# aszepieniec/stark-anatomy

Hardware: NVIDIA H100
Metric: 128-bit field butterflies/sec on 2^20 NTT (higher is better)
Workload: dtype u128 mod p (4x u32 limbs, Montgomery)

## Files before the change

### stark-anatomy_b200/csrc/ntt_tile.cuh

```cuda
#pragma once
#include "field.cuh"

namespace sa {

constexpr int TILE_MAX_PEERS = 7;

struct TileArgs {
    const fe *in;
    fe *out;
    const fe *tw;
    const fe *twb;
    long long in_sr, in_sc, in_sb;
    long long out_sr, out_sc, out_sb;
    long long twb_stride;
    long long in_sb2, out_sb2;
    int inner;
    int ncols;
    int nbatch;
    int has_scale;
    fe scale;
    fe cst[8];
    fe *peer_out[TILE_MAX_PEERS];
    int npeer;
    fe *mc_out;
};

enum { TF_FULL = 1, TF_TWB = 2, TF_SCALE = 4, TF_DYNAMIC = 8, TF_PEERS = 16 };

template <int LOGL, int ELOG, int C>
struct TilePlan {
    static constexpr int L = 1 << LOGL;
    static constexpr int EL = LOGL >= ELOG ? ELOG : LOGL;
    static constexpr int E = 1 << EL;
    static constexpr int NFULL = LOGL / EL;
    static constexpr int REM = LOGL % EL;
    static constexpr int NST = NFULL + (REM ? 1 : 0);
    static constexpr int NLOOP = NST - 1;
    static constexpr int LASTLOG = REM ? REM : EL;
    static constexpr int TPT = (L / E) * C;
    static constexpr int TPC = TPT >= 128 ? 1 : 128 / TPT;
    static constexpr int THREADS = TPT * TPC;
    static constexpr size_t TILE_BYTES = (size_t)TPC * L * C * sizeof(fe);
    static constexpr size_t TW_BYTES = (size_t)L * sizeof(fe);
    SA_HDC size_t smem_bytes() { return NST > 1 ? TILE_BYTES + TW_BYTES + 16 : 0; }
};

SA_HDC int tile_tw_slot(int e) { return e ^ ((e >> 3) & 7); }

SA_HDC int tile_bitrev(int i, int r) {
    int j = 0;
    for (int b = 1, bb = r >> 1; b < r; b <<= 1, bb >>= 1)
        if (i & b) j |= bb;
    return j;
}

template <int R, int LEN>
SA_HD void dft_level(fe *x, const fe *cst, int cstep) {
    constexpr int HALF = LEN / 2, STEP = R / LEN;
#if defined(__CUDA_ARCH__)
#pragma unroll
#endif
    for (int g = 0; g < R; g += LEN) {
#if defined(__CUDA_ARCH__)
#pragma unroll
#endif
        for (int k = 0; k < HALF; k++) {
            const fe t = (k == 0) ? x[g + k + HALF] : fe_montmul(x[g + k + HALF], cst[k * STEP * cstep]);
            const fe e = x[g + k];
            x[g + k] = fe_add(e, t);
            x[g + k + HALF] = fe_sub(e, t);
        }
    }
    if constexpr (LEN < R) dft_level<R, LEN * 2>(x, cst, cstep);
}

template <int R>
SA_HD void dft_regs(fe *x, const fe *cst, int cstep) {
#if defined(__CUDA_ARCH__)
#pragma unroll
#endif
// ... 58 lines not shown
#endif
}

SA_HD long long tile_batch_offset(long long b, int inner, long long sb, long long sb2) {
    return inner <= 1 ? b * sb : (b / inner) * sb + (b % inner) * sb2;
}

#if defined(__CUDA_ARCH__)
__device__ __forceinline__ void tile_stage_twiddles(fe *dst, const fe *src, uint32_t bytes, uint64_t *bar) {
    const uint32_t bar_a = (uint32_t)__cvta_generic_to_shared(bar);
    const uint32_t dst_a = (uint32_t)__cvta_generic_to_shared(dst);
    asm volatile("mbarrier.init.shared::cta.b64 [%0], 1;" ::"r"(bar_a));
    asm volatile("fence.mbarrier_init.release.cluster;" ::: "memory");
    asm volatile("mbarrier.arrive.expect_tx.shared::cta.b64 _, [%0], %1;" ::"r"(bar_a), "r"(bytes) : "memory");
    asm volatile("cp.async.bulk.shared::cluster.global.mbarrier::complete_tx::bytes [%0], [%1], %2, [%3];" ::"r"(dst_a),
                 "l"(src), "r"(bytes), "r"(bar_a)
                 : "memory");
}
__device__ __forceinline__ void tile_wait_twiddles(uint64_t *bar) {
    const uint32_t bar_a = (uint32_t)__cvta_generic_to_shared(bar);
    asm volatile(
        "{\n\t"
        ".reg .pred p;\n\t"
        "TW_WAIT_%=:\n\t"
        "mbarrier.try_wait.parity.shared::cta.b64 p, [%0], 0;\n\t"
        "@p bra TW_DONE_%=;\n\t"
        "bra TW_WAIT_%=;\n\t"
        "TW_DONE_%=:\n\t"
        "}" ::"r"(bar_a)
        : "memory");
}
#endif

template <int LOGL, int ELOG, int C, int FLAGS>
SA_HD void ntt_tile_full_stage(int t, fe *sm, const TileArgs &a, long long b, int col0, bool valid, bool first,
                               int ml, const fe *tw, uint64_t *bar) {
    using P = TilePlan<LOGL, ELOG, C>;
    constexpr int R = P::E;
    constexpr int CSTEP = 16 / R;
    const int c = t % C, q = t / C;
    const int col = col0 + c;
    const bool active = (FLAGS & TF_FULL) ? true : (valid && col < a.ncols);
    const int M = 1 << ml, wlog = LOGL - ml - P::EL;
    const int K = q >> ml, m = q & (M - 1);
    const int row0 = (K << (ml + P::EL)) + m;
    fe x[R];
    if (first) {
        const fe *src = a.in + tile_batch_offset(b, a.inner, a.in_sb, a.in_sb2) + (long long)col * a.in_sc;
        const unsigned sr = (unsigned)a.in_sr, step = (unsigned)M * sr, off0 = (unsigned)row0 * sr;
#if defined(__CUDA_ARCH__)
#pragma unroll
#endif
        for (int d = 0; d < R; d++) x[d] = active ? tile_ld(src + (off0 + (unsigned)d * step)) : fe_zero();
    } else {
#if defined(__CUDA_ARCH__)
#pragma unroll
#endif
        for (int d = 0; d < R; d++) x[d] = tile_ld(sm + (row0 + d * M) * C + c);
    }
    dft_regs<R>(x, a.cst, CSTEP);
#if defined(__CUDA_ARCH__)
    extern __shared__ uint4 sa_smem_u4[];
    tw = reinterpret_cast<const fe *>(sa_smem_u4) + P::TILE_BYTES / sizeof(fe);
    if (first) tile_wait_twiddles(reinterpret_cast<uint64_t *>(const_cast<fe *>(tw) + P::L));
    (void)bar;
#else
    (void)bar;
#endif
    tile_st(sm + row0 * C + c, x[0]);
#if defined(__CUDA_ARCH__)
#pragma unroll
#endif
    for (int k = 1; k < R; k++) {
        const fe w = tile_ld(tw + tile_tw_slot((k * m) << wlog));
        tile_st(sm + (row0 + k * M) * C + c, fe_montmul(x[k], w));
    }
}

template <int LOGL, int ELOG, int C, int FLAGS>
SA_HD void ntt_tile_last_stage(int t, fe *sm, const TileArgs &a, long long b, int col0, bool valid) {
    using P = TilePlan<LOGL, ELOG, C>;
    constexpr int R = 1 << P::LASTLOG, U = P::E / R;
    constexpr bool FIRST = P::NST == 1;
    constexpr int CSTEP = LOGL >= 4 ? 16 / R : (1 << LOGL) / R;
    const int c = t % C, q = t / C;
    const int col = col0 + c;
    const bool active = (FLAGS & TF_FULL) ? true : (valid && col < a.ncols);
    const bool use_twb = (FLAGS & TF_DYNAMIC) ? (a.twb != nullptr) : ((FLAGS & TF_TWB) != 0);
    const bool use_scale = (FLAGS & TF_DYNAMIC) ? (a.has_scale != 0) : ((FLAGS & TF_SCALE) != 0);
    const fe *twb = use_twb ? a.twb + col : nullptr;
    const unsigned out_sr = (unsigned)a.out_sr, twb_sr = (unsigned)a.twb_stride;
    fe *dst = a.out + tile_batch_offset(b, a.inner, a.out_sb, a.out_sb2) + (long long)col * a.out_sc;
#if defined(__CUDA_ARCH__)
#pragma unroll 1
#endif
    for (int s = 0; s < U; s++) {
        const int row0 = (q * U + s) * R;
        fe x[R];
        if (FIRST) {
            const fe *src = a.in + tile_batch_offset(b, a.inner, a.in_sb, a.in_sb2) + (long long)col * a.in_sc;
#if defined(__CUDA_ARCH__)
#pragma unroll
#endif
            for (int d = 0; d < R; d++) x[d] = active ? tile_ld(src + (unsigned)(row0 + d) * (unsigned)a.in_sr) : fe_zero();
        } else {
#if defined(__CUDA_ARCH__)
#pragma unroll
#endif
            for (int d = 0; d < R; d++) x[d] = tile_ld(sm + (row0 + d) * C + c);
        }
        dft_regs<R>(x, a.cst, CSTEP);
#if defined(__CUDA_ARCH__)
#pragma unroll
#endif
        for (int k = 0; k < R; k++) {
            const unsigned o = (unsigned)tile_digit_reverse<LOGL, ELOG, C>(row0 + k);
            fe v = x[k];
            if (use_twb && active) v = fe_montmul(v, tile_ldg(twb + o * twb_sr));
            if (use_scale) v = fe_montmul(v, a.scale);
            if (active) {
                if constexpr ((FLAGS & TF_PEERS) != 0) {
                    const long long rel = (dst - a.out) + (long long)(o * out_sr);
                    if (a.mc_out != nullptr) {
                        tile_st_multicast(a.mc_out + rel, v);
                    } else {
                        tile_st(dst + o * out_sr, v);
                        for (int pi = 0; pi < a.npeer; pi++) tile_st(a.peer_out[pi] + rel, v);
                    }
                } else {
                    tile_st(dst + o * out_sr, v);
                }
            }
        }
    }
}

template <int LOGL, int ELOG, int C, int FLAGS = TF_DYNAMIC>
struct TileStages {
    using P = TilePlan<LOGL, ELOG, C>;
    SA_HD static void full(int st, int t, fe *sm, const TileArgs &a, long long b, int col0, bool valid,
                           const fe *tw, uint64_t *bar) {
        ntt_tile_full_stage<LOGL, ELOG, C, FLAGS>(t, sm, a, b, col0, valid, st == 0, LOGL - (st + 1) * P::EL, tw,
                                                   bar);
    }
    SA_HD static void last(int t, fe *sm, const TileArgs &a, long long b, int col0, bool valid) {
        ntt_tile_last_stage<LOGL, ELOG, C, FLAGS>(t, sm, a, b, col0, valid);
    }
};

template <int LOGL, int ELOG, int C>
SA_HD int tile_variant(const TileArgs &a) {
    using P = TilePlan<LOGL, ELOG, C>;
    const long long tiles = (long long)((a.ncols + C - 1) / C) * a.nbatch;
    const int peers = (a.npeer > 0 || a.mc_out != nullptr) ? TF_PEERS : 0;
    if (LOGL < 5 || a.ncols % C != 0 || tiles % P::TPC != 0 || a.has_scale) return TF_DYNAMIC | peers;
    if (peers) return a.twb == nullptr ? (TF_FULL | TF_PEERS) : (TF_DYNAMIC | TF_PEERS);
    return TF_FULL | (a.twb != nullptr ? TF_TWB : 0);
}

}
```

### stark-anatomy_b200/csrc/sa_b200.cu

```cuda
#include <cuda_runtime.h>
#include <pthread.h>
#include <sched.h>

#include <algorithm>
#include <atomic>
#include <cctype>
#include <chrono>
#include <cstdio>
#include <cstdlib>
#include <cstring>
#include <map>
#include <memory>
#include <mutex>
#include <string>
#include <tuple>
#include <vector>

#include "../../include/sa_b200.h"
#include "field.cuh"
#include "fri_merkle.cuh"
#include "hash.cuh"
#include "ntt_plan.cuh"
#include "ntt_tile.cuh"

// ... 26 lines not shown
}
static inline bool host_is_pow2(size_t n) { return n && !(n & (n - 1)); }
static inline int host_log2(size_t n) {
    int l = 0;
    while ((size_t(1) << l) < n) l++;
    return l;
}

template <int LOGL, int ELOG, int C>
struct TileLaunch {
    using P = TilePlan<LOGL, ELOG, C>;
    static constexpr int TARGET = (P::EL <= 3 && LOGL > 3) ? 1024 : 512;
    static constexpr int MINB = TARGET / P::THREADS > 0 ? TARGET / P::THREADS : 1;
};

template <int LOGL, int ELOG, int C, int FLAGS>
__global__ void __launch_bounds__(TilePlan<LOGL, ELOG, C>::THREADS, TileLaunch<LOGL, ELOG, C>::MINB)
    ntt_tile_kernel(const __grid_constant__ TileArgs a, long long total_tiles, int tiles_per_batch) {
    using P = TilePlan<LOGL, ELOG, C>;
    using S = TileStages<LOGL, ELOG, C, FLAGS>;
    extern __shared__ uint4 sa_smem_u4[];
    fe *smem = reinterpret_cast<fe *>(sa_smem_u4);
    const int tic = threadIdx.x / P::TPT, t = threadIdx.x % P::TPT;
    const long long tile = (long long)blockIdx.x * P::TPC + tic;
    const bool valid = tile < total_tiles;
    const long long b = valid ? tile / tiles_per_batch : 0;
    const int col0 = valid ? (int)(tile % tiles_per_batch) * C : 0;
    fe *sm = smem + (size_t)tic * P::L * C;
    fe *tw = nullptr;
    uint64_t *bar = nullptr;
    asm volatile("griddepcontrol.launch_dependents;");
    if constexpr (P::NLOOP > 0) {
        tw = smem + P::TILE_BYTES / sizeof(fe);
        bar = reinterpret_cast<uint64_t *>(tw + P::L);
        if (threadIdx.x == 0) tile_stage_twiddles(tw, a.tw, (uint32_t)P::TW_BYTES, bar);
        __syncthreads();
    }
    asm volatile("griddepcontrol.wait;" ::: "memory");
#pragma unroll 1
    for (int st = 0; st < P::NLOOP; st++) {
        S::full(st, t, sm, a, b, col0, valid, tw, bar);
        __syncthreads();
    }
    S::last(t, sm, a, b, col0, valid);
}

__global__ void k_pow_table(fe *out, fe base_m, fe lead_m, long long count, int swz) {
    const long long e0 = ((long long)blockIdx.x * blockDim.x + threadIdx.x) * 16;
    if (e0 >= count) return;
    fe acc = fe_montmul(fe_mont_pow_u64(base_m, (uint64_t)e0), lead_m);
    for (int i = 0; i < 16 && e0 + i < count; i++) {
        const long long e = e0 + i;
        tile_st(out + (swz ? (long long)tile_tw_slot((int)e) : e), acc);
        acc = fe_montmul(acc, base_m);
    }
}
__global__ void k_twb_table(fe *out, fe w_m, fe scale_m, int n1, int n2) {
    const long long idx = (long long)blockIdx.x * blockDim.x + threadIdx.x;
    const long long per_row = (n2 + 15) / 16;
    const long long k = idx / per_row;
    const long long j0 = (idx % per_row) * 16;
    if (k >= n1) return;
    const fe wk = fe_mont_pow_u64(w_m, (uint64_t)k);
    fe acc = fe_montmul(fe_mont_pow_u64(wk, (uint64_t)j0), scale_m);
    for (int i = 0; i < 16 && j0 + i < n2; i++) {
        tile_st(out + k * n2 + j0 + i, acc);
        acc = fe_montmul(acc, wk);
    }
}

__global__ void k_pointwise_mul(fe *out, const fe *a, const fe *b, long long n) {
    const long long stride = (long long)gridDim.x * blockDim.x;
    for (long long i = (long long)blockIdx.x * blockDim.x + threadIdx.x; i < n; i += stride)
        tile_st(out + i, fe_montmul(fe_to_mont(tile_ld(a + i)), tile_ld(b + i)));
}
__global__ void k_pointwise_div(fe *out, const fe *a, const fe *b, long long n, int *zero_flag) {
    constexpr int G = 8;
    const long long stride = (long long)gridDim.x * blockDim.x;
    const long long i0 = (long long)blockIdx.x * blockDim.x + threadIdx.x;
    for (long long base = i0; base < n; base += stride * G) {
        fe bm[G], pre[G];
        fe acc = fe_mont_one();
#pragma unroll
        for (int g = 0; g < G; g++) {
            const long long i = base + g * stride;
            fe v = (i < n) ? tile_ld(b + i) : fe_one();
            if (fe_is_zero(v)) {
                *zero_flag = 1;
// ... 681 lines not shown
            if (it->second.tick < victim->second.tick) victim = it;
        g_cache_bytes -= victim->second.tables->bytes;
        g_cache.erase(victim);
    }
}
template <class T>
static std::shared_ptr<T> cache_find(const CacheKey &key) {
    cache_config();
    std::lock_guard<std::mutex> lock(g_plan_mu);
    auto it = g_cache.find(key);
    if (it == g_cache.end()) return nullptr;
    it->second.tick = ++g_cache_tick;
    return std::static_pointer_cast<T>(it->second.tables);
}
template <class T>
static std::shared_ptr<T> cache_publish(const CacheKey &key, std::shared_ptr<T> made) {
    std::lock_guard<std::mutex> lock(g_plan_mu);
    auto it = g_cache.find(key);
    if (it != g_cache.end()) {
        it->second.tick = ++g_cache_tick;
        return std::static_pointer_cast<T>(it->second.tables);
    }
    cache_make_room(made->bytes);
    CacheEntry e;
    e.tables = made;
    e.tick = ++g_cache_tick;
    g_cache.emplace(key, e);
    g_cache_bytes += made->bytes;
    return made;
}

static int build_pow_table(DeviceTables &owner, fe **out, const fe &base_m, const fe &lead_m, long long count,
                           cudaStream_t st, int swz = 0) {
    int rc = owner.alloc((void **)out, sizeof(fe) * (size_t)count);
    if (rc != SA_OK) return rc;
    const long long threads = (count + 15) / 16;
    const int bs = 128;
    k_pow_table<<<(unsigned)((threads + bs - 1) / bs), bs, 0, st>>>(*out, base_m, lead_m, count, swz);
    SA_LAUNCH_CHECK();
    return SA_OK;
}

static int get_plan(PlanPtr *plan_out, int log_n, const fe &root, int inverse, cudaStream_t st) {
    int dev = 0;
    SA_CUDA(cudaGetDevice(&dev));
    const uint64_t rlo = (uint64_t)root.v[0] | ((uint64_t)root.v[1] << 32);
    const uint64_t rhi = (uint64_t)root.v[2] | ((uint64_t)root.v[3] << 32);
    const CacheKey key(0, dev, (uint64_t)log_n, rlo, rhi, inverse ? 1 : 0);
    if ((*plan_out = cache_find<NttPlan>(key))) return SA_OK;
    const uint64_t n = 1ull << log_n;
    const fe root_m = fe_to_mont(root);
    if (!fe_eq(fe_mont_pow_u64(root_m, n), fe_mont_one())) return SA_EROOTORDER;
    if (fe_eq(fe_mont_pow_u64(root_m, n / 2), fe_mont_one())) return SA_ENOTPRIM;
    const fe w_m = inverse ? fe_mont_inv(root_m) : root_m;
    const fe ninv_m = fe_mont_inv(fe_to_mont(fe_from_u64(n)));
    PlanPtr made = std::make_shared<NttPlan>();
    NttPlan &p = *made;
    p.device = dev;
    p.log_n = log_n;
    int rc;
    const NttShape shape = ntt_shape(log_n);
    p.l1 = shape.l1;
    p.l2 = shape.l2;
    p.l3 = shape.l3;
    if (shape.l3 > 0) {
        const int n1 = 1 << p.l1, n2 = 1 << p.l2, n3 = 1 << p.l3;
        const long long m = (long long)n2 * n3;
        const fe w1_m = fe_mont_pow_u64(w_m, (uint64_t)m);
        const fe wsub_m = fe_mont_pow_u64(w_m, (uint64_t)n1);
        const fe w2_m = fe_mont_pow_u64(wsub_m, (uint64_t)n3);
        const fe w3_m = fe_mont_pow_u64(wsub_m, (uint64_t)n2);
        if ((rc = build_pow_table(p, &p.tw1, w1_m, fe_mont_one(), n1, st, 1)) != SA_OK) return rc;
// ... 73 lines not shown
    const int tiles_per_batch = (a.ncols + C - 1) / C;
    const long long total = (long long)tiles_per_batch * a.nbatch;
    const long long grid = (total + P::TPC - 1) / P::TPC;
    const size_t smem = P::smem_bytes();
    if (smem > 48 * 1024) {
        static std::atomic<bool> attr_done[SA_MAX_DEVICES];
        const int rc = optin_smem(ntt_tile_kernel<LOGL, ELOG, C, FLAGS>, attr_done, smem);
        if (rc != SA_OK) return rc;
    }
    static const bool pdl = !(getenv("SA_NTT_PDL") && atoi(getenv("SA_NTT_PDL")) == 0);
    if (pdl) {
        cudaLaunchConfig_t cfg = {};
        cfg.gridDim = dim3((unsigned)grid);
        cfg.blockDim = dim3(P::THREADS);
        cfg.dynamicSmemBytes = smem;
        cfg.stream = st;
        cudaLaunchAttribute attr[1];
        attr[0].id = cudaLaunchAttributeProgrammaticStreamSerialization;
        attr[0].val.programmaticStreamSerializationAllowed = 1;
        cfg.attrs = attr;
        cfg.numAttrs = 1;
        const int tpb = tiles_per_batch;
        SA_CUDA(cudaLaunchKernelEx(&cfg, ntt_tile_kernel<LOGL, ELOG, C, FLAGS>, a, total, tpb));
        g_launches.fetch_add(1, std::memory_order_relaxed);
        return SA_OK;
    }
    ntt_tile_kernel<LOGL, ELOG, C, FLAGS><<<(unsigned)grid, P::THREADS, smem, st>>>(a, total, tiles_per_batch);
    SA_LAUNCH_CHECK();
    return SA_OK;
}
template <int LOGL, int ELOG, int C>
static int launch_tile(const TileArgs &a, cudaStream_t st) {
    const int variant = tile_variant<LOGL, ELOG, C>(a);
    if constexpr (LOGL >= 5) {
        switch (variant) {
            case TF_FULL | TF_TWB: return launch_tile_variant<LOGL, ELOG, C, TF_FULL | TF_TWB>(a, st);
            case TF_FULL: return launch_tile_variant<LOGL, ELOG, C, TF_FULL>(a, st);
            case TF_FULL | TF_PEERS: return launch_tile_variant<LOGL, ELOG, C, TF_FULL | TF_PEERS>(a, st);
        }
    }
    if (variant & TF_PEERS) return launch_tile_variant<LOGL, ELOG, C, TF_DYNAMIC | TF_PEERS>(a, st);
    return launch_tile_variant<LOGL, ELOG, C, TF_DYNAMIC>(a, st);
}

static int g_tile_elog = -1, g_tile_c = -1;
static void tile_config() {
    if (g_tile_elog >= 0) return;
    const char *e = getenv("SA_NTT_ELOG"), *c = getenv("SA_NTT_C");
    g_tile_elog = e ? atoi(e) : 0;
    g_tile_c = c ? atoi(c) : 0;
}
template <int LOGL>
static int launch_tile_shape(const TileArgs &a, cudaStream_t st) {
    tile_config();
#ifdef SA_TUNE
    if (LOGL >= 9 && g_tile_elog > 0) {
        if (g_tile_elog == 3 && g_tile_c == 8) return launch_tile<LOGL, 3, 8>(a, st);
        if (g_tile_elog == 3 && g_tile_c == 4) return launch_tile<LOGL, 3, 4>(a, st);
        if (g_tile_elog == 3 && g_tile_c == 2) return launch_tile<LOGL, 3, 2>(a, st);
        if (g_tile_elog == 4 && g_tile_c == 4) return launch_tile<LOGL, 4, 4>(a, st);
        if (g_tile_elog == 4 && g_tile_c == 2) return launch_tile<LOGL, 4, 2>(a, st);
        if (g_tile_elog == 4 && g_tile_c == 8) return launch_tile<LOGL, 4, 8>(a, st);
    }
#endif
    if constexpr (LOGL >= 9) {
        static const int peer_c = [] {
// ... 1226 lines not shown
```

### stark-anatomy_b200/csrc/field.cuh

```cuda
#pragma once
#include <stdint.h>

#if defined(__CUDACC__)
#define SA_HD __host__ __device__ __forceinline__
#define SA_HDC __host__ __device__ static constexpr
#define SA_ALIGN16 __align__(16)
#else
#define SA_HD inline
#define SA_HDC static constexpr
#define SA_ALIGN16 alignas(16)
#endif

namespace sa {

struct SA_ALIGN16 fe {
    uint32_t v[4];
};

static constexpr uint32_t P3 = 0xCB800000u;

SA_HD fe fe_make(uint32_t a0, uint32_t a1, uint32_t a2, uint32_t a3) {
    fe r;
    r.v[0] = a0; r.v[1] = a1; r.v[2] = a2; r.v[3] = a3;
    return r;
// ... 102 lines not shown
    uint32_t ca = (uint32_t)(s >> 63);
    uint32_t cb = (u0 != 0u);
    u = (u >> 32) + (uint64_t)m1 * P3;
    uint32_t u1 = (uint32_t)u;
    u = (u >> 32) + (uint64_t)m2 * P3;
    uint32_t u2 = (uint32_t)u;
    u = (u >> 32) + (uint64_t)m3 * P3;
    uint32_t u3 = (uint32_t)u;
    uint32_t u4 = (uint32_t)(u >> 32);
    c = (uint64_t)t[4] + u1 + ca + cb;
    uint32_t r0 = (uint32_t)c;
    c = (c >> 32) + t[5] + u2;
    uint32_t r1 = (uint32_t)c;
    c = (c >> 32) + t[6] + u3;
    uint32_t r2 = (uint32_t)c;
    c = (c >> 32) + t[7] + u4;
    uint32_t r3 = (uint32_t)c;
    return fe_cond_sub_p_portable(r0, r1, r2, r3, (uint32_t)(c >> 32));
}

#if defined(__CUDA_ARCH__) && !defined(SA_PORTABLE_FIELD)
__device__ __forceinline__ fe fe_cond_sub_p(uint32_t r0, uint32_t r1, uint32_t r2, uint32_t r3, uint32_t top) {
    uint32_t d0, d1, d2, d3, br;
    asm("sub.cc.u32 %0, %5, 1;\n\t"
        "subc.cc.u32 %1, %6, 0;\n\t"
        "subc.cc.u32 %2, %7, 0;\n\t"
        "subc.cc.u32 %3, %8, 0xCB800000;\n\t"
        "subc.u32 %4, 0, 0;"
        : "=r"(d0), "=r"(d1), "=r"(d2), "=r"(d3), "=r"(br)
        : "r"(r0), "r"(r1), "r"(r2), "r"(r3));
    bool use = (top != 0) | (br == 0);
    return fe_make(use ? d0 : r0, use ? d1 : r1, use ? d2 : r2, use ? d3 : r3);
}
#ifndef SA_FIELD_MASK
#define SA_FIELD_MASK 1
#endif
#ifndef SA_MONTMUL_V
#define SA_MONTMUL_V 1
#endif
template <bool ALU_MASKS>
__device__ __forceinline__ fe fe_cond_add_p(uint32_t d0, uint32_t d1, uint32_t d2, uint32_t d3, uint32_t m) {
    uint32_t p0, p3;
    if (ALU_MASKS) {
        p0 = m & 1u;
        p3 = m & 0xCB800000u;
    } else {
        asm("mul.lo.u32 %0, %2, %2;\n\t"
            "mul.lo.u32 %1, %2, 0x34800000;"
            : "=r"(p0), "=r"(p3) : "r"(m));
    }
    uint32_t r0, r1, r2, r3;
    asm("add.cc.u32 %0, %4, %8;\n\t"
        "addc.cc.u32 %1, %5, 0;\n\t"
        "addc.cc.u32 %2, %6, 0;\n\t"
        "addc.u32 %3, %7, %9;"
        : "=r"(r0), "=r"(r1), "=r"(r2), "=r"(r3)
        : "r"(d0), "r"(d1), "r"(d2), "r"(d3), "r"(p0), "r"(p3));
    return fe_make(r0, r1, r2, r3);
}
__device__ __forceinline__ fe fe_add(const fe &a, const fe &b) {
    uint32_t s0, s1, s2, s3, c;
    asm("add.cc.u32 %0, %5, %9;\n\t"
        "addc.cc.u32 %1, %6, %10;\n\t"
        "addc.cc.u32 %2, %7, %11;\n\t"
        "addc.cc.u32 %3, %8, %12;\n\t"
        "addc.u32 %4, 0, 0;"
        : "=r"(s0), "=r"(s1), "=r"(s2), "=r"(s3), "=r"(c)
        : "r"(a.v[0]), "r"(a.v[1]), "r"(a.v[2]), "r"(a.v[3]), "r"(b.v[0]), "r"(b.v[1]), "r"(b.v[2]),
          "r"(b.v[3]));
    return fe_cond_sub_p(s0, s1, s2, s3, c);
}
__device__ __forceinline__ fe fe_sub(const fe &a, const fe &b) {
    uint32_t d0, d1, d2, d3, m;
    asm("sub.cc.u32 %0, %5, %9;\n\t"
        "subc.cc.u32 %1, %6, %10;\n\t"
        "subc.cc.u32 %2, %7, %11;\n\t"
        "subc.cc.u32 %3, %8, %12;\n\t"
        "subc.u32 %4, 0, 0;"
        : "=r"(d0), "=r"(d1), "=r"(d2), "=r"(d3), "=r"(m)
        : "r"(a.v[0]), "r"(a.v[1]), "r"(a.v[2]), "r"(a.v[3]), "r"(b.v[0]), "r"(b.v[1]), "r"(b.v[2]),
          "r"(b.v[3]));
    return fe_cond_add_p<((SA_FIELD_MASK) >> 2) & 1>(d0, d1, d2, d3, m);
}
__device__ __forceinline__ fe fe_montmul(const fe &a, const fe &b) {
    uint32_t a0 = a.v[0], a1 = a.v[1], a2 = a.v[2], a3 = a.v[3];
    uint32_t b0 = b.v[0], b1 = b.v[1], b2 = b.v[2], b3 = b.v[3];
    uint32_t e0, e1, e2, e3, e4, e5, e6, e7, o0, o1, o2, o3, o4, o5, o6;
    asm("{\n\t"
        "mul.lo.u32 %0, %15, %19;\n\t"
        "mul.hi.u32 %1, %15, %19;\n\t"
        "mul.lo.u32 %2, %15, %21;\n\t"
        "mul.hi.u32 %3, %15, %21;\n\t"
        "mul.lo.u32 %8, %15, %20;\n\t"
        "mul.hi.u32 %9, %15, %20;\n\t"
        "mul.lo.u32 %10, %15, %22;\n\t"
        "mul.hi.u32 %11, %15, %22;\n\t"
        "mad.lo.cc.u32 %2, %16, %20, %2;\n\t"
        "madc.hi.cc.u32 %3, %16, %20, %3;\n\t"
        "madc.lo.cc.u32 %4, %16, %22, 0;\n\t"
        "madc.hi.u32 %5, %16, %22, 0;\n\t"
        "mad.lo.cc.u32 %8, %16, %19, %8;\n\t"
        "madc.hi.cc.u32 %9, %16, %19, %9;\n\t"
        "madc.lo.cc.u32 %10, %16, %21, %10;\n\t"
        "madc.hi.cc.u32 %11, %16, %21, %11;\n\t"
        "addc.u32 %12, 0, 0;\n\t"
        "mad.lo.cc.u32 %2, %17, %19, %2;\n\t"
        "madc.hi.cc.u32 %3, %17, %19, %3;\n\t"
        "madc.lo.cc.u32 %4, %17, %21, %4;\n\t"
        "madc.hi.cc.u32 %5, %17, %21, %5;\n\t"
        "addc.u32 %6, 0, 0;\n\t"
        "mad.lo.cc.u32 %10, %17, %20, %10;\n\t"
        "madc.hi.cc.u32 %11, %17, %20, %11;\n\t"
        "madc.lo.cc.u32 %12, %17, %22, %12;\n\t"
        "madc.hi.u32 %13, %17, %22, 0;\n\t"
        "mad.lo.cc.u32 %4, %18, %20, %4;\n\t"
        "madc.hi.cc.u32 %5, %18, %20, %5;\n\t"
        "madc.lo.cc.u32 %6, %18, %22, %6;\n\t"
        "madc.hi.u32 %7, %18, %22, 0;\n\t"
        "mad.lo.cc.u32 %10, %18, %19, %10;\n\t"
        "madc.hi.cc.u32 %11, %18, %19, %11;\n\t"
        "madc.lo.cc.u32 %12, %18, %21, %12;\n\t"
        "madc.hi.cc.u32 %13, %18, %21, %13;\n\t"
        "addc.u32 %14, 0, 0;\n\t"
        "add.cc.u32 %1, %1, %8;\n\t"
        "addc.cc.u32 %2, %2, %9;\n\t"
        "addc.cc.u32 %3, %3, %10;\n\t"
        "addc.cc.u32 %4, %4, %11;\n\t"
        "addc.cc.u32 %5, %5, %12;\n\t"
        "addc.cc.u32 %6, %6, %13;\n\t"
        "addc.u32 %7, %7, %14;\n\t"
        "}"
        : "=&r"(e0), "=&r"(e1), "=&r"(e2), "=&r"(e3), "=&r"(e4), "=&r"(e5), "=&r"(e6), "=&r"(e7),
          "=&r"(o0), "=&r"(o1), "=&r"(o2), "=&r"(o3), "=&r"(o4), "=&r"(o5), "=&r"(o6)
        : "r"(a0), "r"(a1), "r"(a2), "r"(a3), "r"(b0), "r"(b1), "r"(b2), "r"(b3));
    (void)o0; (void)o1; (void)o2; (void)o3; (void)o4; (void)o5; (void)o6;
#if SA_MONTMUL_V >= 2
    {
        uint32_t x = e0 * P3;
        uint32_t m3, nw;
        asm("sub.cc.u32 %0, %2, %3;\n\t"
            "subc.u32 %1, 0, 0;"
            : "=r"(m3), "=r"(nw)
            : "r"(e3), "r"(x));
        uint32_t E0, E1, E2, E3, O0, O1, O2, O3;
        asm("mul.lo.u32 %0, %8, 0xCB800000;\n\t"
            "mul.hi.u32 %1, %8, 0xCB800000;\n\t"
            "mul.lo.u32 %2, %10, 0xCB800000;\n\t"
            "mul.hi.u32 %3, %10, 0xCB800000;\n\t"
            "mul.lo.u32 %4, %9, 0xCB800000;\n\t"
            "mul.hi.u32 %5, %9, 0xCB800000;\n\t"
            "mul.lo.u32 %6, %11, 0xCB800000;\n\t"
            "mul.hi.u32 %7, %11, 0xCB800000;"
            : "=r"(E0), "=r"(E1), "=r"(E2), "=r"(E3), "=r"(O0), "=r"(O1), "=r"(O2), "=r"(O3)
            : "r"(e0), "r"(e1), "r"(e2), "r"(m3));
        (void)E0;
        O0 |= nw & 1u;
        uint32_t r0, r1, r2, r3, ta, tb;
        asm("sub.cc.u32 %0, %5, %9;\n\t"
            "subc.cc.u32 %1, %6, %10;\n\t"
            "subc.cc.u32 %2, %7, %11;\n\t"
            "subc.cc.u32 %3, %8, 0;\n\t"
            "subc.u32 %4, 0, 0;"
            : "=r"(r0), "=r"(r1), "=r"(r2), "=r"(r3), "=r"(ta)
            : "r"(e4), "r"(e5), "r"(e6), "r"(e7), "r"(E1), "r"(E2), "r"(E3));
        asm("sub.cc.u32 %0, %0, %5;\n\t"
            "subc.cc.u32 %1, %1, %6;\n\t"
            "subc.cc.u32 %2, %2, %7;\n\t"
            "subc.cc.u32 %3, %3, %8;\n\t"
            "subc.u32 %4, 0, 0;"
            : "+r"(r0), "+r"(r1), "+r"(r2), "+r"(r3), "=r"(tb)
            : "r"(O0), "r"(O1), "r"(O2), "r"(O3));
        return fe_cond_add_p<true>(r0, r1, r2, r3, ta | tb);
    }
#endif
    uint32_t x = e0 * P3;
    uint32_t m3, nw;
    asm("sub.cc.u32 %0, %2, %3;\n\t"
        "subc.u32 %1, 0, 0;"
        : "=r"(m3), "=r"(nw)
        : "r"(e3), "r"(x));
    uint32_t w;
    if ((SA_FIELD_MASK) & 1)
        w = nw & 1u;
    else
        asm("mul.lo.u32 %0, %1, %1;" : "=r"(w) : "r"(nw));
    uint32_t u1, u2, u3, u4;
    asm("mad.hi.u32 %0, %4, 0xCB800000, %8;\n\t"
        "mad.lo.cc.u32 %0, %5, 0xCB800000, %0;\n\t"
        "madc.hi.u32 %1, %5, 0xCB800000, 0;\n\t"
        "mad.lo.cc.u32 %1, %6, 0xCB800000, %1;\n\t"
        "madc.hi.u32 %2, %6, 0xCB800000, 0;\n\t"
        "mad.lo.cc.u32 %2, %7, 0xCB800000, %2;\n\t"
        "madc.hi.u32 %3, %7, 0xCB800000, 0;"
        : "=&r"(u1), "=&r"(u2), "=&r"(u3), "=&r"(u4)
        : "r"(e0), "r"(e1), "r"(e2), "r"(m3), "r"(w));
    uint32_t r0, r1, r2, r3, top;
    asm("sub.cc.u32 %0, %5, %9;\n\t"
        "subc.cc.u32 %1, %6, %10;\n\t"
        "subc.cc.u32 %2, %7, %11;\n\t"
        "subc.cc.u32 %3, %8, %12;\n\t"
        "subc.u32 %4, 0, 0;"
        : "=r"(r0), "=r"(r1), "=r"(r2), "=r"(r3), "=r"(top)
        : "r"(e4), "r"(e5), "r"(e6), "r"(e7), "r"(u1), "r"(u2), "r"(u3), "r"(u4));
    return fe_cond_add_p<((SA_FIELD_MASK) >> 1) & 1>(r0, r1, r2, r3, top);
}
#else
SA_HD fe fe_add(const fe &a, const fe &b) { return fe_add_portable(a, b); }
SA_HD fe fe_sub(const fe &a, const fe &b) { return fe_sub_portable(a, b); }
SA_HD fe fe_montmul(const fe &a, const fe &b) { return fe_montmul_portable(a, b); }
#endif
SA_HD fe fe_neg(const fe &a) { return fe_sub(fe_zero(), a); }

SA_HD fe fe_to_mont(const fe &a) { return fe_montmul(a, fe_r2()); }
SA_HD fe fe_from_mont(const fe &a) { return fe_montmul(a, fe_one()); }
SA_HD fe fe_mul(const fe &a, const fe &b) { return fe_montmul(fe_to_mont(a), b); }

SA_HD fe fe_mont_pow_u64(const fe &base_m, uint64_t e) {
    fe acc = fe_mont_one();
    fe b = base_m;
    while (e) {
        if (e & 1) acc = fe_montmul(acc, b);
        b = fe_montmul(b, b);
        e >>= 1;
    }
    return acc;
}

SA_HD fe fe_mont_inv(const fe &a_m) {
    const uint32_t e[4] = {0xFFFFFFFFu, 0xFFFFFFFFu, 0xFFFFFFFFu, 0xCB7FFFFFu};
    fe acc = fe_mont_one();
    for (int w = 3; w >= 0; w--) {
        for (int bit = 31; bit >= 0; bit--) {
            acc = fe_montmul(acc, acc);
            if ((e[w] >> bit) & 1u) acc = fe_montmul(acc, a_m);
        }
    }
    return acc;
// ... 4 lines not shown
```

Baseline: 190.9 billion.

## Precompute per-row twiddle tables and unroll stages for 1024-point NTT tiles

For 1024-point tiles with radix-16 stages, twiddles are laid out in a precomputed row table (17 entries per m value for each of two stages). Threads then read consecutive shared-memory entries instead of computing swizzled exponent indices. The full-stage loop and the last-stage loop are fully unrolled with compile-time stage indices. The last stage hoists the digit-reverse base offset and preloads the output twiddle factors. A rolled fallback variant is kept for small grids, in exchange for more shared memory, extra register pressure and a larger table build.

```diff
diff --git a/stark-anatomy_b200/csrc/ntt_tile.cuh b/stark-anatomy_b200/csrc/ntt_tile.cuh
--- a/stark-anatomy_b200/csrc/ntt_tile.cuh
+++ b/stark-anatomy_b200/csrc/ntt_tile.cuh
@@ -25,7 +25,15 @@
     fe *mc_out;
 };
 
-enum { TF_FULL = 1, TF_TWB = 2, TF_SCALE = 4, TF_DYNAMIC = 8, TF_PEERS = 16 };
+enum { TF_FULL = 1, TF_TWB = 2, TF_SCALE = 4, TF_DYNAMIC = 8, TF_PEERS = 16, TF_ROLLED = 32 };
+
+constexpr int TILE_ROW = 17;
+constexpr int TILE_ROW_ELEMS = (64 + 4) * TILE_ROW;
+SA_HDC int tile_row_exponent(int i) {
+    const int r = i / TILE_ROW, k = i % TILE_ROW + 1;
+    if (k > 15) return -1;
+    return r < 64 ? k * r : (k * (r - 64)) << 4;
+}
 
 template <int LOGL, int ELOG, int C>
 struct TilePlan {
@@ -40,12 +48,23 @@
     static constexpr int TPT = (L / E) * C;
     static constexpr int TPC = TPT >= 128 ? 1 : 128 / TPT;
     static constexpr int THREADS = TPT * TPC;
+    static constexpr bool ROWS = LOGL == 10 && EL == 4;
+    template <int FLAGS>
+    SA_HDC bool unrolled() {
+        return ROWS && (FLAGS & TF_FULL) != 0 && (FLAGS & (TF_PEERS | TF_ROLLED)) == 0;
+    }
     static constexpr size_t TILE_BYTES = (size_t)TPC * L * C * sizeof(fe);
-    static constexpr size_t TW_BYTES = (size_t)L * sizeof(fe);
+    static constexpr int TW_ELEMS = ROWS ? TILE_ROW_ELEMS : L;
+    static constexpr size_t TW_BYTES = (size_t)TW_ELEMS * sizeof(fe);
     SA_HDC size_t smem_bytes() { return NST > 1 ? TILE_BYTES + TW_BYTES + 16 : 0; }
 };
 
 SA_HDC int tile_tw_slot(int e) { return e ^ ((e >> 3) & 7); }
+
+SA_HD fe tile_row_entry(const fe *tw, int i) {
+    const int e = tile_row_exponent(i);
+    return e < 0 ? fe_zero() : tw[tile_tw_slot(e)];
+}
 
 SA_HDC int tile_bitrev(int i, int r) {
     int j = 0;
@@ -170,12 +189,14 @@
 }
 #endif
 
-template <int LOGL, int ELOG, int C, int FLAGS>
-SA_HD void ntt_tile_full_stage(int t, fe *sm, const TileArgs &a, long long b, int col0, bool valid, bool first,
-                               int ml, const fe *tw, uint64_t *bar) {
+template <int LOGL, int ELOG, int C, int FLAGS, int ST = -1>
+SA_HD void ntt_tile_full_stage(int t, fe *sm, const TileArgs &a, long long b, int col0, bool valid, bool first_rt,
+                               int ml_rt, const fe *tw, uint64_t *bar) {
     using P = TilePlan<LOGL, ELOG, C>;
     constexpr int R = P::E;
     constexpr int CSTEP = 16 / R;
+    const bool first = ST >= 0 ? ST == 0 : first_rt;
+    const int ml = ST >= 0 ? LOGL - (ST + 1) * P::EL : ml_rt;
     const int c = t % C, q = t / C;
     const int col = col0 + c;
     const bool active = (FLAGS & TF_FULL) ? true : (valid && col < a.ncols);
@@ -200,18 +221,29 @@
 #if defined(__CUDA_ARCH__)
     extern __shared__ uint4 sa_smem_u4[];
     tw = reinterpret_cast<const fe *>(sa_smem_u4) + P::TILE_BYTES / sizeof(fe);
-    if (first) tile_wait_twiddles(reinterpret_cast<uint64_t *>(const_cast<fe *>(tw) + P::L));
+    if (first) tile_wait_twiddles(reinterpret_cast<uint64_t *>(const_cast<fe *>(tw) + P::TW_ELEMS));
     (void)bar;
 #else
     (void)bar;
 #endif
     tile_st(sm + row0 * C + c, x[0]);
-#if defined(__CUDA_ARCH__)
-#pragma unroll
-#endif
-    for (int k = 1; k < R; k++) {
-        const fe w = tile_ld(tw + tile_tw_slot((k * m) << wlog));
-        tile_st(sm + (row0 + k * M) * C + c, fe_montmul(x[k], w));
+    if constexpr (P::ROWS) {
+        const int row = (first ? 0 : 64 * TILE_ROW) + m * TILE_ROW - 1;
+#if defined(__CUDA_ARCH__)
+#pragma unroll
+        for (int k = 1; k < R; k++) tile_st(sm + (row0 + k * M) * C + c, fe_montmul(x[k], tile_ld(tw + row + k)));
+#else
+        for (int k = 1; k < R; k++)
+            tile_st(sm + (row0 + k * M) * C + c, fe_montmul(x[k], tile_row_entry(tw, row + k)));
+#endif
+    } else {
+#if defined(__CUDA_ARCH__)
+#pragma unroll
+#endif
+        for (int k = 1; k < R; k++) {
+            const fe w = tile_ld(tw + tile_tw_slot((k * m) << wlog));
+            tile_st(sm + (row0 + k * M) * C + c, fe_montmul(x[k], w));
+        }
     }
 }
 
@@ -229,12 +261,24 @@
     const fe *twb = use_twb ? a.twb + col : nullptr;
     const unsigned out_sr = (unsigned)a.out_sr, twb_sr = (unsigned)a.twb_stride;
     fe *dst = a.out + tile_batch_offset(b, a.inner, a.out_sb, a.out_sb2) + (long long)col * a.out_sc;
-#if defined(__CUDA_ARCH__)
-#pragma unroll 1
+    const unsigned obase = (unsigned)tile_digit_reverse<LOGL, ELOG, C>(q * P::E);
+    dst += obase * out_sr;
+    if (use_twb) twb += obase * twb_sr;
+    constexpr int UNR = P::template unrolled<FLAGS>() ? U : 1;
+#if defined(__CUDA_ARCH__)
+#pragma unroll UNR
 #endif
     for (int s = 0; s < U; s++) {
         const int row0 = (q * U + s) * R;
-        fe x[R];
+        const unsigned ounit = (unsigned)tile_digit_reverse<LOGL, ELOG, C>(s * R);
+        fe x[R], wb[R];
+        if (use_twb && active) {
+#if defined(__CUDA_ARCH__)
+#pragma unroll
+#endif
+            for (int k = 0; k < R; k++)
+                wb[k] = tile_ldg(twb + (ounit + (unsigned)tile_digit_reverse<LOGL, ELOG, C>(k)) * twb_sr);
+        }
         if (FIRST) {
             const fe *src = a.in + tile_batch_offset(b, a.inner, a.in_sb, a.in_sb2) + (long long)col * a.in_sc;
 #if defined(__CUDA_ARCH__)
@@ -252,9 +296,9 @@
 #pragma unroll
 #endif
         for (int k = 0; k < R; k++) {
-            const unsigned o = (unsigned)tile_digit_reverse<LOGL, ELOG, C>(row0 + k);
+            const unsigned o = ounit + (unsigned)tile_digit_reverse<LOGL, ELOG, C>(k);
             fe v = x[k];
-            if (use_twb && active) v = fe_montmul(v, tile_ldg(twb + o * twb_sr));
+            if (use_twb && active) v = fe_montmul(v, wb[k]);
             if (use_scale) v = fe_montmul(v, a.scale);
             if (active) {
                 if constexpr ((FLAGS & TF_PEERS) != 0) {
@@ -276,10 +320,19 @@
 template <int LOGL, int ELOG, int C, int FLAGS = TF_DYNAMIC>
 struct TileStages {
     using P = TilePlan<LOGL, ELOG, C>;
+    static constexpr bool UNROLL = P::template unrolled<FLAGS>();
     SA_HD static void full(int st, int t, fe *sm, const TileArgs &a, long long b, int col0, bool valid,
                            const fe *tw, uint64_t *bar) {
-        ntt_tile_full_stage<LOGL, ELOG, C, FLAGS>(t, sm, a, b, col0, valid, st == 0, LOGL - (st + 1) * P::EL, tw,
-                                                   bar);
+        if constexpr (UNROLL) {
+            static_assert(P::NLOOP == 2, "the row tables cover two full stages");
+            if (st == 0)
+                ntt_tile_full_stage<LOGL, ELOG, C, FLAGS, 0>(t, sm, a, b, col0, valid, true, 0, tw, bar);
+            else
+                ntt_tile_full_stage<LOGL, ELOG, C, FLAGS, 1>(t, sm, a, b, col0, valid, false, 0, tw, bar);
+        } else {
+            ntt_tile_full_stage<LOGL, ELOG, C, FLAGS>(t, sm, a, b, col0, valid, st == 0, LOGL - (st + 1) * P::EL,
+                                                       tw, bar);
+        }
     }
     SA_HD static void last(int t, fe *sm, const TileArgs &a, long long b, int col0, bool valid) {
         ntt_tile_last_stage<LOGL, ELOG, C, FLAGS>(t, sm, a, b, col0, valid);
diff --git a/stark-anatomy_b200/csrc/sa_b200.cu b/stark-anatomy_b200/csrc/sa_b200.cu
--- a/stark-anatomy_b200/csrc/sa_b200.cu
+++ b/stark-anatomy_b200/csrc/sa_b200.cu
@@ -82,12 +82,13 @@
     asm volatile("griddepcontrol.launch_dependents;");
     if constexpr (P::NLOOP > 0) {
         tw = smem + P::TILE_BYTES / sizeof(fe);
-        bar = reinterpret_cast<uint64_t *>(tw + P::L);
-        if (threadIdx.x == 0) tile_stage_twiddles(tw, a.tw, (uint32_t)P::TW_BYTES, bar);
+        bar = reinterpret_cast<uint64_t *>(tw + P::TW_ELEMS);
+        if (threadIdx.x == 0) tile_stage_twiddles(tw, a.tw + (P::ROWS ? P::L : 0), (uint32_t)P::TW_BYTES, bar);
         __syncthreads();
     }
     asm volatile("griddepcontrol.wait;" ::: "memory");
-#pragma unroll 1
+    constexpr int UNR = S::UNROLL ? P::NLOOP : 1;
+#pragma unroll UNR
     for (int st = 0; st < P::NLOOP; st++) {
         S::full(st, t, sm, a, b, col0, valid, tw, bar);
         __syncthreads();
@@ -104,6 +105,11 @@
         tile_st(out + (swz ? (long long)tile_tw_slot((int)e) : e), acc);
         acc = fe_montmul(acc, base_m);
     }
+}
+__global__ void k_row_table(fe *out, const fe *tw) {
+    const int i = blockIdx.x * blockDim.x + threadIdx.x;
+    if (i >= TILE_ROW_ELEMS) return;
+    tile_st(out + i, tile_row_entry(tw, i));
 }
 __global__ void k_twb_table(fe *out, fe w_m, fe scale_m, int n1, int n2) {
     const long long idx = (long long)blockIdx.x * blockDim.x + threadIdx.x;
@@ -851,12 +857,17 @@
 
 static int build_pow_table(DeviceTables &owner, fe **out, const fe &base_m, const fe &lead_m, long long count,
                            cudaStream_t st, int swz = 0) {
-    int rc = owner.alloc((void **)out, sizeof(fe) * (size_t)count);
+    const bool rows = swz && count == 1024;
+    int rc = owner.alloc((void **)out, sizeof(fe) * (size_t)(count + (rows ? TILE_ROW_ELEMS : 0)));
     if (rc != SA_OK) return rc;
     const long long threads = (count + 15) / 16;
     const int bs = 128;
     k_pow_table<<<(unsigned)((threads + bs - 1) / bs), bs, 0, st>>>(*out, base_m, lead_m, count, swz);
     SA_LAUNCH_CHECK();
+    if (rows) {
+        k_row_table<<<(TILE_ROW_ELEMS + bs - 1) / bs, bs, 0, st>>>(*out + count, *out);
+        SA_LAUNCH_CHECK();
+    }
     return SA_OK;
 }
 
@@ -996,6 +1007,16 @@
 template <int LOGL, int ELOG, int C>
 static int launch_tile(const TileArgs &a, cudaStream_t st) {
     const int variant = tile_variant<LOGL, ELOG, C>(a);
+    if constexpr (TilePlan<LOGL, ELOG, C>::ROWS) {
+        using P = TilePlan<LOGL, ELOG, C>;
+        const long long grid = ((long long)((a.ncols + C - 1) / C) * a.nbatch + P::TPC - 1) / P::TPC;
+        if (grid <= TileLaunch<LOGL, ELOG, C>::MINB * sm_count()) {
+            switch (variant) {
+                case TF_FULL | TF_TWB: return launch_tile_variant<LOGL, ELOG, C, TF_FULL | TF_TWB | TF_ROLLED>(a, st);
+                case TF_FULL: return launch_tile_variant<LOGL, ELOG, C, TF_FULL | TF_ROLLED>(a, st);
+            }
+        }
+    }
     if constexpr (LOGL >= 5) {
         switch (variant) {
             case TF_FULL | TF_TWB: return launch_tile_variant<LOGL, ELOG, C, TF_FULL | TF_TWB>(a, st);
```

Result: faster. 195.0 billion, median of 6 (+2.2%).

## Rewrite Montgomery multiply with even/odd product split and fused single-word reduction

Applied to the files above, without the earlier changes.

Replaces the 4-limb schoolbook product with a separate even/odd partial-product accumulation using PTX-local registers, then applies a new single-asm reduction that exploits the special prime form (p = 0xCB800000·2^96 + 1) to subtract the multiples of p in one carry chain. It also removes the compile-time mask variants and always builds the conditional-add masks with multiplies instead of ALU ANDs. The intent is a shorter dependency chain and fewer instructions per montmul in the NTT butterfly. The risks are wrong carry handling in the reduction and extra multiply pressure from the mask multiplies.

```diff
diff --git a/stark-anatomy_b200/csrc/field.cuh b/stark-anatomy_b200/csrc/field.cuh
--- a/stark-anatomy_b200/csrc/field.cuh
+++ b/stark-anatomy_b200/csrc/field.cuh
@@ -158,23 +158,11 @@
     bool use = (top != 0) | (br == 0);
     return fe_make(use ? d0 : r0, use ? d1 : r1, use ? d2 : r2, use ? d3 : r3);
 }
-#ifndef SA_FIELD_MASK
-#define SA_FIELD_MASK 1
-#endif
-#ifndef SA_MONTMUL_V
-#define SA_MONTMUL_V 1
-#endif
-template <bool ALU_MASKS>
 __device__ __forceinline__ fe fe_cond_add_p(uint32_t d0, uint32_t d1, uint32_t d2, uint32_t d3, uint32_t m) {
     uint32_t p0, p3;
-    if (ALU_MASKS) {
-        p0 = m & 1u;
-        p3 = m & 0xCB800000u;
-    } else {
-        asm("mul.lo.u32 %0, %2, %2;\n\t"
-            "mul.lo.u32 %1, %2, 0x34800000;"
-            : "=r"(p0), "=r"(p3) : "r"(m));
-    }
+    asm("mul.lo.u32 %0, %2, %2;\n\t"
+        "mul.lo.u32 %1, %2, 0x34800000;"
+        : "=r"(p0), "=r"(p3) : "r"(m));
     uint32_t r0, r1, r2, r3;
     asm("add.cc.u32 %0, %4, %8;\n\t"
         "addc.cc.u32 %1, %5, 0;\n\t"
@@ -206,129 +194,88 @@
         : "=r"(d0), "=r"(d1), "=r"(d2), "=r"(d3), "=r"(m)
         : "r"(a.v[0]), "r"(a.v[1]), "r"(a.v[2]), "r"(a.v[3]), "r"(b.v[0]), "r"(b.v[1]), "r"(b.v[2]),
           "r"(b.v[3]));
-    return fe_cond_add_p<((SA_FIELD_MASK) >> 2) & 1>(d0, d1, d2, d3, m);
+    return fe_cond_add_p(d0, d1, d2, d3, m);
 }
 __device__ __forceinline__ fe fe_montmul(const fe &a, const fe &b) {
-    uint32_t a0 = a.v[0], a1 = a.v[1], a2 = a.v[2], a3 = a.v[3];
-    uint32_t b0 = b.v[0], b1 = b.v[1], b2 = b.v[2], b3 = b.v[3];
-    uint32_t e0, e1, e2, e3, e4, e5, e6, e7, o0, o1, o2, o3, o4, o5, o6;
+    uint32_t t0, t1, t2, t3, t4, t5, t6, t7;
     asm("{\n\t"
-        "mul.lo.u32 %0, %15, %19;\n\t"
-        "mul.hi.u32 %1, %15, %19;\n\t"
-        "mul.lo.u32 %2, %15, %21;\n\t"
-        "mul.hi.u32 %3, %15, %21;\n\t"
-        "mul.lo.u32 %8, %15, %20;\n\t"
-        "mul.hi.u32 %9, %15, %20;\n\t"
-        "mul.lo.u32 %10, %15, %22;\n\t"
-        "mul.hi.u32 %11, %15, %22;\n\t"
-        "mad.lo.cc.u32 %2, %16, %20, %2;\n\t"
-        "madc.hi.cc.u32 %3, %16, %20, %3;\n\t"
-        "madc.lo.cc.u32 %4, %16, %22, 0;\n\t"
-        "madc.hi.u32 %5, %16, %22, 0;\n\t"
-        "mad.lo.cc.u32 %8, %16, %19, %8;\n\t"
-        "madc.hi.cc.u32 %9, %16, %19, %9;\n\t"
-        "madc.lo.cc.u32 %10, %16, %21, %10;\n\t"
-        "madc.hi.cc.u32 %11, %16, %21, %11;\n\t"
-        "addc.u32 %12, 0, 0;\n\t"
-        "mad.lo.cc.u32 %2, %17, %19, %2;\n\t"
-        "madc.hi.cc.u32 %3, %17, %19, %3;\n\t"
-        "madc.lo.cc.u32 %4, %17, %21, %4;\n\t"
-        "madc.hi.cc.u32 %5, %17, %21, %5;\n\t"
-        "addc.u32 %6, 0, 0;\n\t"
-        "mad.lo.cc.u32 %10, %17, %20, %10;\n\t"
-        "madc.hi.cc.u32 %11, %17, %20, %11;\n\t"
-        "madc.lo.cc.u32 %12, %17, %22, %12;\n\t"
-        "madc.hi.u32 %13, %17, %22, 0;\n\t"
-        "mad.lo.cc.u32 %4, %18, %20, %4;\n\t"
-        "madc.hi.cc.u32 %5, %18, %20, %5;\n\t"
-        "madc.lo.cc.u32 %6, %18, %22, %6;\n\t"
-        "madc.hi.u32 %7, %18, %22, 0;\n\t"
-        "mad.lo.cc.u32 %10, %18, %19, %10;\n\t"
-        "madc.hi.cc.u32 %11, %18, %19, %11;\n\t"
-        "madc.lo.cc.u32 %12, %18, %21, %12;\n\t"
-        "madc.hi.cc.u32 %13, %18, %21, %13;\n\t"
-        "addc.u32 %14, 0, 0;\n\t"
-        "add.cc.u32 %1, %1, %8;\n\t"
-        "addc.cc.u32 %2, %2, %9;\n\t"
-        "addc.cc.u32 %3, %3, %10;\n\t"
-        "addc.cc.u32 %4, %4, %11;\n\t"
-        "addc.cc.u32 %5, %5, %12;\n\t"
-        "addc.cc.u32 %6, %6, %13;\n\t"
-        "addc.u32 %7, %7, %14;\n\t"
+        ".reg .u32 e0, e1, e2, e3, e4, e5, e6, e7, o1, o2, o3, o4, o5, o6, o7;\n\t"
+        "mul.lo.u32 e0, %8, %12;\n\t"
+        "mul.hi.u32 e1, %8, %12;\n\t"
+        "mul.lo.u32 e2, %8, %14;\n\t"
+        "mul.hi.u32 e3, %8, %14;\n\t"
+        "mad.lo.cc.u32 e2, %9, %13, e2;\n\t"
+        "madc.hi.cc.u32 e3, %9, %13, e3;\n\t"
+        "madc.lo.cc.u32 e4, %9, %15, 0;\n\t"
+        "madc.hi.u32 e5, %9, %15, 0;\n\t"
+        "mad.lo.cc.u32 e2, %10, %12, e2;\n\t"
+        "madc.hi.cc.u32 e3, %10, %12, e3;\n\t"
+        "madc.lo.cc.u32 e4, %10, %14, e4;\n\t"
+        "madc.hi.cc.u32 e5, %10, %14, e5;\n\t"
+        "madc.lo.cc.u32 e6, %11, %15, 0;\n\t"
+        "madc.hi.u32 e7, %11, %15, 0;\n\t"
+        "mad.lo.cc.u32 e4, %11, %13, e4;\n\t"
+        "madc.hi.cc.u32 e5, %11, %13, e5;\n\t"
+        "addc.cc.u32 e6, e6, 0;\n\t"
+        "addc.u32 e7, e7, 0;\n\t"
+        "mul.lo.u32 o1, %8, %13;\n\t"
+        "mul.hi.u32 o2, %8, %13;\n\t"
+        "mul.lo.u32 o3, %8, %15;\n\t"
+        "mul.hi.u32 o4, %8, %15;\n\t"
+        "mad.lo.cc.u32 o1, %9, %12, o1;\n\t"
+        "madc.hi.cc.u32 o2, %9, %12, o2;\n\t"
+        "madc.lo.cc.u32 o3, %9, %14, o3;\n\t"
+        "madc.hi.cc.u32 o4, %9, %14, o4;\n\t"
+        "madc.lo.cc.u32 o5, %10, %15, 0;\n\t"
+        "madc.hi.u32 o6, %10, %15, 0;\n\t"
+        "mad.lo.cc.u32 o3, %10, %13, o3;\n\t"
+        "madc.hi.cc.u32 o4, %10, %13, o4;\n\t"
+        "madc.lo.cc.u32 o5, %11, %14, o5;\n\t"
+        "madc.hi.cc.u32 o6, %11, %14, o6;\n\t"
+        "addc.u32 o7, 0, 0;\n\t"
+        "mad.lo.cc.u32 o3, %11, %12, o3;\n\t"
+        "madc.hi.cc.u32 o4, %11, %12, o4;\n\t"
+        "addc.cc.u32 o5, o5, 0;\n\t"
+        "addc.cc.u32 o6, o6, 0;\n\t"
+        "addc.u32 o7, o7, 0;\n\t"
+        "mov.u32 %0, e0;\n\t"
+        "add.cc.u32 %1, e1, o1;\n\t"
+        "addc.cc.u32 %2, e2, o2;\n\t"
+        "addc.cc.u32 %3, e3, o3;\n\t"
+        "addc.cc.u32 %4, e4, o4;\n\t"
+        "addc.cc.u32 %5, e5, o5;\n\t"
+        "addc.cc.u32 %6, e6, o6;\n\t"
+        "addc.u32 %7, e7, o7;\n\t"
         "}"
-        : "=&r"(e0), "=&r"(e1), "=&r"(e2), "=&r"(e3), "=&r"(e4), "=&r"(e5), "=&r"(e6), "=&r"(e7),
-          "=&r"(o0), "=&r"(o1), "=&r"(o2), "=&r"(o3), "=&r"(o4), "=&r"(o5), "=&r"(o6)
-        : "r"(a0), "r"(a1), "r"(a2), "r"(a3), "r"(b0), "r"(b1), "r"(b2), "r"(b3));
-    (void)o0; (void)o1; (void)o2; (void)o3; (void)o4; (void)o5; (void)o6;
-#if SA_MONTMUL_V >= 2
-    {
-        uint32_t x = e0 * P3;
-        uint32_t m3, nw;
-        asm("sub.cc.u32 %0, %2, %3;\n\t"
-            "subc.u32 %1, 0, 0;"
-            : "=r"(m3), "=r"(nw)
-            : "r"(e3), "r"(x));
-        uint32_t E0, E1, E2, E3, O0, O1, O2, O3;
-        asm("mul.lo.u32 %0, %8, 0xCB800000;\n\t"
-            "mul.hi.u32 %1, %8, 0xCB800000;\n\t"
-            "mul.lo.u32 %2, %10, 0xCB800000;\n\t"
-            "mul.hi.u32 %3, %10, 0xCB800000;\n\t"
-            "mul.lo.u32 %4, %9, 0xCB800000;\n\t"
-            "mul.hi.u32 %5, %9, 0xCB800000;\n\t"
-            "mul.lo.u32 %6, %11, 0xCB800000;\n\t"
-            "mul.hi.u32 %7, %11, 0xCB800000;"
-            : "=r"(E0), "=r"(E1), "=r"(E2), "=r"(E3), "=r"(O0), "=r"(O1), "=r"(O2), "=r"(O3)
-            : "r"(e0), "r"(e1), "r"(e2), "r"(m3));
-        (void)E0;
-        O0 |= nw & 1u;
-        uint32_t r0, r1, r2, r3, ta, tb;
-        asm("sub.cc.u32 %0, %5, %9;\n\t"
-            "subc.cc.u32 %1, %6, %10;\n\t"
-            "subc.cc.u32 %2, %7, %11;\n\t"
-            "subc.cc.u32 %3, %8, 0;\n\t"
-            "subc.u32 %4, 0, 0;"
-            : "=r"(r0), "=r"(r1), "=r"(r2), "=r"(r3), "=r"(ta)
-            : "r"(e4), "r"(e5), "r"(e6), "r"(e7), "r"(E1), "r"(E2), "r"(E3));
-        asm("sub.cc.u32 %0, %0, %5;\n\t"
-            "subc.cc.u32 %1, %1, %6;\n\t"
-            "subc.cc.u32 %2, %2, %7;\n\t"
-            "subc.cc.u32 %3, %3, %8;\n\t"
-            "subc.u32 %4, 0, 0;"
-            : "+r"(r0), "+r"(r1), "+r"(r2), "+r"(r3), "=r"(tb)
-            : "r"(O0), "r"(O1), "r"(O2), "r"(O3));
-        return fe_cond_add_p<true>(r0, r1, r2, r3, ta | tb);
-    }
-#endif
-    uint32_t x = e0 * P3;
-    uint32_t m3, nw;
-    asm("sub.cc.u32 %0, %2, %3;\n\t"
-        "subc.u32 %1, 0, 0;"
-        : "=r"(m3), "=r"(nw)
-        : "r"(e3), "r"(x));
-    uint32_t w;
-    if ((SA_FIELD_MASK) & 1)
-        w = nw & 1u;
-    else
-        asm("mul.lo.u32 %0, %1, %1;" : "=r"(w) : "r"(nw));
-    uint32_t u1, u2, u3, u4;
-    asm("mad.hi.u32 %0, %4, 0xCB800000, %8;\n\t"
-        "mad.lo.cc.u32 %0, %5, 0xCB800000, %0;\n\t"
-        "madc.hi.u32 %1, %5, 0xCB800000, 0;\n\t"
-        "mad.lo.cc.u32 %1, %6, 0xCB800000, %1;\n\t"
-        "madc.hi.u32 %2, %6, 0xCB800000, 0;\n\t"
-        "mad.lo.cc.u32 %2, %7, 0xCB800000, %2;\n\t"
-        "madc.hi.u32 %3, %7, 0xCB800000, 0;"
-        : "=&r"(u1), "=&r"(u2), "=&r"(u3), "=&r"(u4)
-        : "r"(e0), "r"(e1), "r"(e2), "r"(m3), "r"(w));
-    uint32_t r0, r1, r2, r3, top;
-    asm("sub.cc.u32 %0, %5, %9;\n\t"
-        "subc.cc.u32 %1, %6, %10;\n\t"
-        "subc.cc.u32 %2, %7, %11;\n\t"
-        "subc.cc.u32 %3, %8, %12;\n\t"
-        "subc.u32 %4, 0, 0;"
-        : "=r"(r0), "=r"(r1), "=r"(r2), "=r"(r3), "=r"(top)
-        : "r"(e4), "r"(e5), "r"(e6), "r"(e7), "r"(u1), "r"(u2), "r"(u3), "r"(u4));
-    return fe_cond_add_p<((SA_FIELD_MASK) >> 1) & 1>(r0, r1, r2, r3, top);
+        : "=r"(t0), "=r"(t1), "=r"(t2), "=r"(t3), "=r"(t4), "=r"(t5), "=r"(t6), "=r"(t7)
+        : "r"(a.v[0]), "r"(a.v[1]), "r"(a.v[2]), "r"(a.v[3]), "r"(b.v[0]), "r"(b.v[1]), "r"(b.v[2]),
+          "r"(b.v[3]));
+    uint32_t s0, s1, s2, s3, m;
+    asm("{\n\t"
+        ".reg .u32 x, h0, m3, u0, u1, u2, u3, v1, v2;\n\t"
+        "mul.lo.u32 x, %5, 0xCB800000;\n\t"
+        "mul.hi.u32 h0, %5, 0xCB800000;\n\t"
+        "mul.lo.u32 v1, %7, 0xCB800000;\n\t"
+        "mul.hi.u32 v2, %7, 0xCB800000;\n\t"
+        "mul.lo.u32 u0, %6, 0xCB800000;\n\t"
+        "mul.hi.u32 u1, %6, 0xCB800000;\n\t"
+        "sub.cc.u32 m3, %8, x;\n\t"
+        "subc.cc.u32 %0, %9, h0;\n\t"
+        "subc.cc.u32 %1, %10, v1;\n\t"
+        "subc.cc.u32 %2, %11, v2;\n\t"
+        "subc.cc.u32 %3, %12, 0;\n\t"
+        "subc.u32 %4, 0, 0;\n\t"
+        "mul.lo.u32 u2, m3, 0xCB800000;\n\t"
+        "mul.hi.u32 u3, m3, 0xCB800000;\n\t"
+        "sub.cc.u32 %0, %0, u0;\n\t"
+        "subc.cc.u32 %1, %1, u1;\n\t"
+        "subc.cc.u32 %2, %2, u2;\n\t"
+        "subc.cc.u32 %3, %3, u3;\n\t"
+        "subc.u32 %4, %4, 0;\n\t"
+        "}"
+        : "=&r"(s0), "=&r"(s1), "=&r"(s2), "=&r"(s3), "=&r"(m)
+        : "r"(t0), "r"(t1), "r"(t2), "r"(t3), "r"(t4), "r"(t5), "r"(t6), "r"(t7));
+    return fe_cond_add_p(s0, s1, s2, s3, m);
 }
 #else
 SA_HD fe fe_add(const fe &a, const fe &b) { return fe_add_portable(a, b); }
```

New measurement: 182.7 billion before, 184.2 billion after (median of 6 runs). Within noise of the previous version (+0.8%).
